# jianwang-mpi/GlobalEgoMocap

Hardware: AMD Instinct MI355X
Metric: optimised windows/sec (10-frame, 15-joint) (higher is better)
Workload: dtype f32

## Files before the change

### __graft_entry__.py

```python
import os
import subprocess
import sys

ROOT = os.path.dirname(os.path.abspath(__file__))
if ROOT not in sys.path:
    sys.path.insert(0, ROOT)

CSRC = os.path.join(ROOT, "globalegomocap_amd", "csrc")
LIB_DIR = os.path.join(ROOT, "globalegomocap_amd", "_lib")
LIB = os.path.join(LIB_DIR, "libgem_hip.so")
SOURCES = ["gem_api.hip", "weights.hip", "stage.hip", "gemm_f32.hip", "gemm_bf16.hip", "decoder_bf16.hip", "energy.hip", "lbfgs.hip", "tail.hip", "tail_bf16.hip", "train.hip", "errors.hip", "chunk_io.hip"]


def _stale():
    if not os.path.exists(LIB):
        return True
    t = os.path.getmtime(LIB)
    deps = [os.path.join(CSRC, f) for f in os.listdir(CSRC)] + [os.path.join(ROOT, "include", "gem_hip.h"),
                                                                os.path.abspath(__file__)]
    return any(os.path.getmtime(d) > t for d in deps)


NO_PACKED_FP32 = ["-Xclang", "-target-feature", "-Xclang", "-packed-fp32-ops", "-DGEM_NO_PACKED_FP32"]
FP_CONTRACT = ["-ffp-contract=on"]
EXTRA_FLAGS = {}
OBJ_DIR = os.path.join(ROOT, "build", "obj")
# ... 172 lines not shown
```

### globalegomocap_amd/csrc/energy.hip

```cpp
#include "energy_device.h"

namespace gem {

__global__ void pack_pose_kernel(const float* __restrict__ src, float* __restrict__ dst, int rows, int C) {
    const int i = blockIdx.x * blockDim.x + threadIdx.x;
    if (i >= rows * PAD) return;
    const int r = i / PAD, c = i % PAD;
    dst[i] = c < C ? src[(size_t)r * C + c] : 0.f;
}
__global__ void unpack_pose_kernel(const float* __restrict__ src, float* __restrict__ dst, int rows, int C) {
    const int i = blockIdx.x * blockDim.x + threadIdx.x;
    if (i >= rows * C) return;
    const int r = i / C, c = i % C;
    dst[i] = src[(size_t)r * PAD + c];
}
int launch_pack_pose(const float* src, float* dst, int rows, int C, hipStream_t s) {
    const int n = rows * PAD;
    hipLaunchKernelGGL(pack_pose_kernel, dim3((n + 255) / 256), dim3(256), 0, s, src, dst, rows, C);
    GEM_HIP(hipGetLastError());
    return 0;
}
int launch_unpack_pose(const float* src, float* dst, int rows, int C, hipStream_t s) {
    const int n = rows * C;
    hipLaunchKernelGGL(unpack_pose_kernel, dim3((n + 255) / 256), dim3(256), 0, s, src, dst, rows, C);
    GEM_HIP(hipGetLastError());
    return 0;
}

__global__ void reparam_kernel(const float* __restrict__ mulv, const float* __restrict__ eps, float* mu, float* logvar,
                               float* z, float* z2, int B, int D, int Dp) {
    const int i = blockIdx.x * blockDim.x + threadIdx.x;
    if (i >= B * Dp) return;
    const int b = i / Dp, k = i % Dp;
    float m = 0.f, lv = 0.f, zz = 0.f;
    if (k < D) {
        m = mulv[(size_t)b * 2 * Dp + k];
        lv = mulv[(size_t)b * 2 * Dp + Dp + k];
        zz = eps ? eps[(size_t)b * D + k] * expf(0.5f * lv) + m : m;
        if (mu) mu[(size_t)b * D + k] = m;
        if (logvar) logvar[(size_t)b * D + k] = lv;
        if (z) z[(size_t)b * D + k] = zz;
    }
    if (z2) z2[i] = zz;
}
int launch_reparam(const float* mulv, const float* eps, float* mu, float* logvar, float* z, float* z2, int B, int D, int Dp,
                   hipStream_t s) {
    const int n = B * Dp;
    hipLaunchKernelGGL(reparam_kernel, dim3((n + 255) / 256), dim3(256), 0, s, mulv, eps, mu, logvar, z, z2, B, D, Dp);
    GEM_HIP(hipGetLastError());
    return 0;
}
__global__ void pad_latent_kernel(const float* __restrict__ z, float* __restrict__ zp, int B, int D, int Dp) {
    const int i = blockIdx.x * blockDim.x + threadIdx.x;
// ... 81 lines not shown

__global__ void gather_windows_kernel(const float* __restrict__ frames, const int32_t* __restrict__ frame0,
                                      float* __restrict__ out, int B, int T, int JC) {
    const int i = blockIdx.x * blockDim.x + threadIdx.x;
    if (i >= B * T * JC) return;
    const int b = i / (T * JC), r = i - b * T * JC;
    out[i] = frames[(size_t)frame0[b] * JC + r];
}
int launch_gather_windows(const float* frames, const int32_t* frame0, float* out, int B, int T, int JC, hipStream_t s) {
    const int n = B * T * JC;
    hipLaunchKernelGGL(gather_windows_kernel, dim3((n + 255) / 256), dim3(256), 0, s, frames, frame0, out, B, T, JC);
    GEM_HIP(hipGetLastError());
    return 0;
}

__device__ void inv4_rigid_general(const double* m, double* o) {
    const double a = m[0], b = m[1], c = m[2], d = m[4], e = m[5], f = m[6], g = m[8], hh = m[9], i = m[10];
    const double A = e * i - f * hh, Bc = -(d * i - f * g), Cc = d * hh - e * g;
    const double det = a * A + b * Bc + c * Cc;
    const double id = 1.0 / det;
    double r[9] = {A * id, -(b * i - c * hh) * id, (b * f - c * e) * id,
                   Bc * id, (a * i - c * g) * id, -(a * f - c * d) * id,
                   Cc * id, -(a * hh - b * g) * id, (a * e - b * d) * id};
    const double tx = m[3], ty = m[7], tz = m[11];
    for (int q = 0; q < 3; ++q) {
        o[q * 4 + 0] = r[q * 3 + 0]; o[q * 4 + 1] = r[q * 3 + 1]; o[q * 4 + 2] = r[q * 3 + 2];
        o[q * 4 + 3] = -(r[q * 3 + 0] * tx + r[q * 3 + 1] * ty + r[q * 3 + 2] * tz);
    }
    o[12] = 0; o[13] = 0; o[14] = 0; o[15] = 1;
}

__global__ __launch_bounds__(64) void relative_global_kernel(const float* __restrict__ local, const double* __restrict__ cams,
                                                             const int32_t* __restrict__ frame0, float* __restrict__ rel,
                                                             int T, int J) {
    __shared__ double M[MAXT][12];
    const int b = blockIdx.x, lane = threadIdx.x;
    const double* c0 = cams + (size_t)frame0[b] * 16;
    if (lane < T) {
        double inv0[16];
        inv4_rigid_general(c0, inv0);
        const double* ct = c0 + (size_t)lane * 16;
        for (int r = 0; r < 3; ++r)
            for (int c = 0; c < 4; ++c) {
                double acc = 0;
                for (int k = 0; k < 4; ++k) acc += inv0[r * 4 + k] * ct[k * 4 + c];
                M[lane][r * 4 + c] = acc;
            }
    }
    __syncthreads();
    for (int p = lane; p < T * J; p += 64) {
        const int t = p / J;
        const float* x = local + ((size_t)b * T * J + p) * 3;
        const double X = x[0], Y = x[1], Z = x[2];
        float* o = rel + ((size_t)b * T * J + p) * 3;
        for (int r = 0; r < 3; ++r)
            o[r] = (float)(M[t][r * 4 + 0] * X + M[t][r * 4 + 1] * Y + M[t][r * 4 + 2] * Z + M[t][r * 4 + 3]);
    }
}
__global__ __launch_bounds__(64) void to_global_kernel(const float* __restrict__ rel, const double* __restrict__ cams,
                                                       const int32_t* __restrict__ frame0, double* __restrict__ out, int T, int J) {
    const int b = blockIdx.x, lane = threadIdx.x;
    const double* c0 = cams + (size_t)frame0[b] * 16;
    for (int p = lane; p < T * J; p += 64) {
        const float* x = rel + ((size_t)b * T * J + p) * 3;
        const double X = x[0], Y = x[1], Z = x[2];
        double* o = out + ((size_t)b * T * J + p) * 3;
        for (int r = 0; r < 3; ++r) o[r] = c0[r * 4 + 0] * X + c0[r * 4 + 1] * Y + c0[r * 4 + 2] * Z + c0[r * 4 + 3];
    }
}
int launch_relative_global(const float* local, const double* cams, const int32_t* frame0, float* rel, int B, int T, int J,
                           hipStream_t s) {
    hipLaunchKernelGGL(relative_global_kernel, dim3(B), dim3(64), 0, s, local, cams, frame0, rel, T, J);
    GEM_HIP(hipGetLastError());
    return 0;
}
int launch_to_global(const float* rel, const double* cams, const int32_t* frame0, double* out, int B, int T, int J,
                     hipStream_t s) {
    hipLaunchKernelGGL(to_global_kernel, dim3(B), dim3(64), 0, s, rel, cams, frame0, out, T, J);
    GEM_HIP(hipGetLastError());
    return 0;
}

}
// ... 1 lines not shown
```

### globalegomocap_amd/csrc/gem_internal.h

```cpp
#pragma once
#if defined(__HIP_DEVICE_COMPILE__) && !defined(GEM_NO_PACKED_FP32)
#error "compile with: -Xclang -target-feature -Xclang -packed-fp32-ops -DGEM_NO_PACKED_FP32 (__graft_entry__.NO_PACKED_FP32)"
#endif

#include <hip/hip_runtime.h>
#include <stdint.h>
#include <atomic>
#include <set>
#include <string>
#include <vector>

#include "../../include/gem_hip.h"

namespace gem {

constexpr int PAD = 64;
constexpr float LEAKY_SLOPE = 0.01f;
constexpr double BN_EPS = 1e-5;
constexpr int MAX_HIST = 128;
constexpr int MAXJ_ERR = GEM_MAX_JOINTS;
constexpr int N_LOG = 1 << 16;
constexpr int TRACE_ROUNDS = 64;

inline int pad64(int x) { return (x + PAD - 1) / PAD * PAD; }
// ... 77 lines not shown
    double* parts = nullptr;
    int* tex_key = nullptr;
    float* tex_val = nullptr;
    double* trace = nullptr;
    float* pose_a = nullptr;
    float* pose_b = nullptr;
    float* splitk = nullptr;
    size_t splitk_elems = 0;
    int* perm = nullptr;
    int* slot_of = nullptr;
    int* n_active = nullptr;
    int *perm2 = nullptr, *slot_of2 = nullptr;
    int* n_log = nullptr;
    long log_pos = 0;
    int done_phase = 3;
    int dbg_slots = -1, dbg_B = 0, dbg_round = 0;
    long dbg_log0 = 0;
    std::vector<void*> allocs;
};

enum Repack {
    REPACK_NONE = 0,
    REPACK_KERNEL = 1,
    REPACK_FUSED = 2,
    REPACK_ATOMIC = 3
};

struct RoundSet {
    int* n_active = nullptr;
    int* perm = nullptr;
// ... 70 lines not shown
}
__device__ __forceinline__ double wave_max_dpp(double v) {
    v = nan_max(v, dpp_move<0xB1>(v));
    v = nan_max(v, dpp_move<0x4E>(v));
    v = nan_max(v, dpp_move<0x141>(v));
    v = nan_max(v, dpp_move<0x140>(v));
    return nan_max(nan_max(nan_max(read_lane(v, 0), read_lane(v, 16)), read_lane(v, 32)), read_lane(v, 48));
}

}

namespace gem {
struct GraphKey {
    int kind = 0, stage = 0, B = 0, precision = 0;
    bool tex_cache = true;
    const void* ptr[12] = {};
    gem_energy_weights w[2] = {};
    gem_lbfgs_opts opt = {};
    void* stream = nullptr;
};
struct GraphEntry {
    GraphKey key;
    hipGraph_t graph = nullptr;
    hipGraphExec_t exec = nullptr;
    uint64_t last_use = 0;
};
}

struct gem_handle {
    gem_config cfg;
// ... 163 lines not shown
int launch_relative_global(const float* local, const double* cams, const int32_t* frame0, float* rel, int B, int T, int J,
                           hipStream_t s);
int launch_to_global(const float* rel, const double* cams, const int32_t* frame0, double* out, int B, int T, int J,
                     hipStream_t s);

int launch_errors(gem_handle* h, const double* est, const double* mid, const double* opt, const double* gt, int F,
                  const double* bone_mm, double* frame_out, double* out, hipStream_t s, int n_seq);
int launch_merge(const double* win, double* tmp, double* out, int n_chunks, int wpc, int T, int JC, int overlap, int smooth,
                 hipStream_t s);
size_t errors_frame_lds_bytes(int J);
void drop_graphs(gem_handle* h);
int post_scratch(gem_handle* h, size_t elems);
int launch_lift(gem_handle* h, const float* heat, const double* depth, int F, const double* poly, int n_poly, int up, int pad_x,
                int pad_y, double* out64, float* out32, hipStream_t s);

int launch_lbfgs_init(gem_handle* h, int B, hipStream_t s);
int launch_lbfgs_advance(gem_handle* h, int B, const gem_lbfgs_opts& o, const RoundSet& rs, const SlabSrc& grad, hipStream_t s);
int launch_lbfgs_stats(gem_handle* h, int B, gem_window_stats* out, hipStream_t s);
int launch_compact(gem_handle* h, const RoundSet& rs, int B, int force_all, hipStream_t s, int zero_after = 0);
int launch_lbfgs_debug_read(gem_handle* h, int B, gem_lbfgs_debug_state* out, float* x, float* d, float* trial, hipStream_t s);


}
```

### globalegomocap_amd/csrc/lbfgs.hip

```cpp
#include "gem_internal.h"

namespace gem {

typedef float f32x4 __attribute__((ext_vector_type(4)));

enum { PH_INIT = 0, PH_BRACKET = 1, PH_ZOOM = 2, PH_DONE = 3 };
static_assert(PH_DONE == 3, "Workspace::done_phase (gem_internal.h) names this value for the fused compaction of gemm_rows.h");

struct AdvArgs {
    LbfgsState* state;
    const double* f;
    double* trace;
    const float* gnew;
    float *x, *d, *g, *gp, *bg0, *bg1, *trial, *S, *Y;
    uint16_t* trial_b;
    int* phase_arr;
    const int* slot_of;
    int *next_perm, *next_slot_of, *next_count;
    SlabSrc gslab;
    unsigned long long* clk;
    int Dp, hist_cap;
    gem_lbfgs_opts o;
};

// ... 563 lines not shown
    }
#endif
    (void)full_path;
#undef LB_PROBE
}

template <int EPT, bool FULL, bool HB = false>
__global__ __launch_bounds__(256) void lbfgs_advance_kernel(AdvArgs a) { lbfgs_advance_body<EPT, 256, FULL, HB>(a); }

__global__ void lbfgs_init_kernel(LbfgsState* st, int* __restrict__ phase_arr, const float* __restrict__ trial, float* __restrict__ x, int B,
                                  int Dp) {
    const size_t i = (size_t)blockIdx.x * blockDim.x + threadIdx.x;
    if (i < (size_t)B * Dp) x[i] = trial[i];
    if (i < (size_t)B) {
        phase_arr[i] = PH_INIT;
        LbfgsState* s = st + i;
        s->phase = PH_INIT; s->n_iter = 0; s->evals = 0; s->ls_iter = 0; s->ls_evals = 0; s->max_ls = 0;
        s->first_bracket = 0; s->ls_done = 0; s->insuf = 0; s->low = 0; s->high = 1; s->hist_count = 0; s->hist_start = 0;
        s->nan_seen = 0;
        s->loss = 0; s->prev_loss = 0; s->t = 0; s->gtd = 0; s->d_norm = 0; s->H_diag = 1;
        s->t_prev = 0; s->f_prev = 0; s->gtd_prev = 0;
        s->br_t[0] = s->br_t[1] = 0; s->br_f[0] = s->br_f[1] = 0; s->br_gtd[0] = s->br_gtd[1] = 0;
    }
}

__global__ void lbfgs_stats_kernel(const LbfgsState* st, gem_window_stats* out, int B) {
    const int i = blockIdx.x * blockDim.x + threadIdx.x;
    if (i >= B) return;
    out[i].n_iter = st[i].n_iter;
    out[i].func_evals = st[i].evals;
    out[i].final_loss = (float)st[i].loss;
    out[i].status = (st[i].phase == PH_DONE ? 1 : 0) | (st[i].nan_seen ? 2 : 0);
}

__global__ __launch_bounds__(256) void lbfgs_debug_read_kernel(const LbfgsState* __restrict__ st, gem_lbfgs_debug_state* __restrict__ out,
                                                               const float* __restrict__ x, const float* __restrict__ d,
                                                               const float* __restrict__ trial, const uint16_t* __restrict__ trial_b,
                                                               float* __restrict__ ox, float* __restrict__ od, float* __restrict__ otrial,
                                                               int D, int Dp) {
    __shared__ int bad;
    const int b = blockIdx.x;
    if (threadIdx.x == 0) bad = 0;
    __syncthreads();
    int mine = 0;
    for (int k = threadIdx.x; k < Dp; k += blockDim.x) {
        const size_t i = (size_t)b * Dp + k;
        const float xv = x[i], dv = d[i];
// ... 137 lines not shown
```

### globalegomocap_amd/csrc/stage.hip

```cpp
#include <cstring>

#include "gem_internal.h"

namespace gem {

__global__ void fill_u32_kernel(uint32_t* __restrict__ p, uint32_t v, size_t n) {
    const size_t i = (size_t)blockIdx.x * blockDim.x + threadIdx.x;
    if (i < n) p[i] = v;
}
static int launch_fill_u32(uint32_t* p, uint32_t v, size_t n, hipStream_t s) {
    if (!n) return 0;
    hipLaunchKernelGGL(fill_u32_kernel, dim3((unsigned)((n + 255) / 256)), dim3(256), 0, s, p, v, n);
    GEM_HIP(hipGetLastError());
    return 0;
}


Route plan_route(const gem_handle* h, int stage, int B, Call call) {
    const StageNet& net = h->net[stage];
    Route rt;
    rt.precision = h->precision;
    const bool bf16 = h->precision == GEM_PRECISION_BF16, have_tail = net.tail_start >= 1;
    const int tail_g = h->T <= 16 ? 16 / h->T : 1;
    rt.tail_wgs = (B + tail_g - 1) / tail_g;
// ... 29 lines not shown
    const bool odd = mode == REPACK_ATOMIC && (k & 1);
    r.perm = odd ? w.perm2 : w.perm;
    r.slot_of = mode == REPACK_NONE ? nullptr : odd ? w.slot_of2 : w.slot_of;
    r.n_active = w.n_active;
    r.log_idx = log0 + k;
    if (mode == REPACK_ATOMIC) {
        r.n_active = w.n_log + (log0 + k) % N_LOG;
        r.next_count = r.n_active + 1;
        r.next_perm = odd ? w.perm : w.perm2;
        r.next_slot_of = odd ? w.slot_of : w.slot_of2;
    }
    r.trace = k < TRACE_ROUNDS ? w.trace + (size_t)k * w.Bmax : nullptr;
    return r;
}

static int begin_rounds(gem_handle* h, int B, int counters, hipStream_t s, long* log0) {
    Workspace& w = h->ws;
    if (counters && (w.log_pos % N_LOG) + counters + 1 > N_LOG) w.log_pos += N_LOG - (w.log_pos % N_LOG);
    *log0 = w.log_pos;
    if (launch_compact(h, round_set(w, *log0, 0, REPACK_KERNEL), B, 1, s, counters)) return 1;
    w.log_pos = *log0 + 1 + counters;
    return 0;
}

static int check_lbfgs_opts(const Workspace& w, const gem_lbfgs_opts& o, const char* who) {
    if (o.max_iter < 1 || o.max_eval < 1 || o.max_iter - 1 > w.hist_cap || o.max_iter > MAX_HIST) {
        set_error(std::string(who) + ": max_iter must be 1.." + std::to_string(w.hist_cap + 1)); return 1;
    }
    if (o.max_eval > 1021) { set_error(std::string(who) + ": max_eval must be at most 1021 (torch's default for max_iter = 25 is 31)"); return 1; }
    return 0;
}

static int check_call(gem_handle* h, int stage, int B, const char* who) {
    if (!h) { set_error(std::string(who) + ": null handle"); return 1; }
    if (stage < 0 || stage > 1 || !h->net[stage].loaded) { set_error(std::string(who) + ": VAE weights of this stage are not loaded"); return 1; }
    if (B < 0 || B > h->ws.Bmax) { set_error(std::string(who) + ": B exceeds max_windows"); return 1; }
    GEM_HIP(hipSetDevice(h->cfg.device));
    return 0;
}

static int encoder_forward(gem_handle* h, int stage, int B, const float* d_pose, hipStream_t s) {
    StageNet& net = h->net[stage];
    Workspace& w = h->ws;
    const int rows = B * h->T;
    if (launch_pack_pose(d_pose, w.pose_p, rows, h->C, s)) return 1;
    const float* in = w.pose_p;
    int lda = PAD;
    for (size_t i = 0; i < net.enc.size(); ++i) {
        if (launch_gemm(h, net.enc[i], EPI_BIAS_LRELU, in, lda, nullptr, w.enc_act[i], net.enc[i].N, rows, h->T, s, -1)) return 1;
        in = w.enc_act[i];
        lda = net.enc[i].N;
    }
    return launch_gemm(h, net.fc, EPI_BIAS, in, net.fc.K, nullptr, w.mulv, net.fc.N, B, h->T, s, -1);
}


static int decoder_forward(gem_handle* h, const Route& rt, int stage, int B, const float* zp, hipStream_t s, const RoundSet* rs = nullptr,
                           int* repack_log = nullptr) {
    StageNet& net = h->net[stage];
    Workspace& w = h->ws;
// ... 98 lines not shown
    fill_tail_args(h, net, rt, B, forward_only, in_slab, ea, rs, &ta);
    ta.g_out = w.dec_grad[st]; ta.g_out_b = nullptr;
    if (launch_tail(h, ta, tail_lds, s, rs)) return 1;
    if (forward_only) return 0;
    return decoder_backward(h, rt, stage, B, s, st - 1, w.dec_grad[st], rs, grad);
}

struct StageRun {
    gem_handle* h = nullptr;
    int stage = 0, B = 0;
    const float* pose_in = nullptr; const float* heat = nullptr; const int32_t* frame0 = nullptr; const float* mean_bone = nullptr;
    const float* eps = nullptr;
    gem_energy_weights wt{}; gem_lbfgs_opts opt{};
    float* pose_out = nullptr; gem_window_stats* stats = nullptr;
    hipStream_t s = nullptr;
    EnergyArgs ea{};
    Route route;
    long log0 = 0;
    int rounds = 0;
};

static int stage_begin(StageRun& r) {
    gem_handle* h = r.h;
    Workspace& w = h->ws;
    const int B = r.B, stage = r.stage;
    hipStream_t s = r.s;
    if (r.wt.reproj != 0.0 && (!r.heat || !r.frame0)) { set_error("optimize: reproj weight != 0 needs heat-maps and frame indices"); return 1; }
    if (check_lbfgs_opts(w, r.opt, "optimize")) return 1;
    r.rounds = r.opt.max_eval + 1;
    w.dbg_slots = -1;
    if (encoder_forward(h, stage, B, r.pose_in, s)) return 1;
    if (launch_reparam(w.mulv, r.eps, nullptr, nullptr, nullptr, w.trial, B, h->D, h->Dp, s)) return 1;
    if (h->precision == GEM_PRECISION_BF16 && launch_f32_to_bf16(w.trial, w.trial_b, (size_t)B * h->Dp, s)) return 1;
    if (launch_lbfgs_init(h, B, s)) return 1;
    r.route = plan_route(h, stage, B, CALL_ROUNDS);
    if (begin_rounds(h, B, r.route.repack == REPACK_ATOMIC ? r.rounds + 1 : 0, s, &r.log0)) return 1;
    const bool tex = h->tex_cache && w.tex_key && r.wt.reproj != 0.0;
    if (tex && launch_fill_u32(reinterpret_cast<uint32_t*>(w.tex_key), 0xFFFFFFFFu, (size_t)B * h->T * h->J, s)) return 1;
    r.ea = energy_args(h, r.pose_in, r.heat, r.frame0, r.mean_bone, r.wt, tex);
    return launch_fill_u32(reinterpret_cast<uint32_t*>(w.trace), 0xFFFFFFFFu, (size_t)TRACE_ROUNDS * w.Bmax * 2, s);
}

static int stage_round(StageRun& r, int k) {
    gem_handle* h = r.h;
    Workspace& w = h->ws;
    const Repack mode = r.route.repack;
    const RoundSet rs = round_set(w, r.log0, k, mode);
    int* repack_log = nullptr;
    if (k > 0 && mode != REPACK_ATOMIC) {
        if (mode == REPACK_FUSED) repack_log = w.n_log + rs.log_idx % N_LOG;
        else if (launch_compact(h, rs, r.B, 0, r.s)) return 1;
        w.log_pos = rs.log_idx + 1;
    }
    r.ea.n_dev = rs.n_active; r.ea.perm = rs.perm;
    SlabSrc grad;
    if (evaluate(h, r.route, r.stage, r.B, w.trial, r.ea, r.s, false, &rs, &grad, repack_log)) return 1;
    return launch_lbfgs_advance(h, r.B, r.opt, rs, grad, r.s);
}

static int stage_finish(StageRun& r) {
    gem_handle* h = r.h;
    Workspace& w = h->ws;
    SlabSrc none;
    if (evaluate(h, r.route, r.stage, r.B, w.trial, energy_args(h, r.pose_in, r.heat, r.frame0, r.mean_bone, r.wt, false), r.s, true, nullptr, &none))
        return 1;
    if (launch_unpack_pose(w.dec_act.back(), r.pose_out, r.B * h->T, h->C, r.s)) return 1;
    if (r.stats && launch_lbfgs_stats(h, r.B, r.stats, r.s)) return 1;
    return 0;
}

static int optimize_stage_impl(gem_handle* h, int stage, int B, const float* d_pose_in, const float* d_heat,
                               const int32_t* d_frame0, const float* d_mean_bone, const float* d_eps,
                               const gem_energy_weights& wt, const gem_lbfgs_opts& opt, float* d_pose_out,
                               gem_window_stats* d_stats, hipStream_t s) {
    StageRun r;
    r.h = h; r.stage = stage; r.B = B; r.pose_in = d_pose_in; r.heat = d_heat; r.frame0 = d_frame0; r.mean_bone = d_mean_bone; r.eps = d_eps;
    r.wt = wt; r.opt = opt; r.pose_out = d_pose_out; r.stats = d_stats; r.s = s;
    int rc = stage_begin(r);
    for (int k = 0; k < r.rounds && !rc; ++k) rc = stage_round(r, k);
    return rc || stage_finish(r);
}

struct WindowsRun {
    gem_handle* h = nullptr;
    int B = 0;
    const float* local_pose = nullptr; const double* cams = nullptr; const float* heat = nullptr; const int32_t* frame0 = nullptr;
    const float* mean_bone = nullptr; const float* eps_local = nullptr; const float* eps_global = nullptr;
    gem_energy_weights w_local{}, w_global{}; gem_lbfgs_opts opt{};
    float* mid_local = nullptr; double* global = nullptr; gem_window_stats* stats_local = nullptr; gem_window_stats* stats_global = nullptr;
    hipStream_t s = nullptr;
    StageRun st;
    float* mid = nullptr;
};

static int windows_begin_local(WindowsRun& r) {
    gem_handle* h = r.h;
    Workspace& w = h->ws;
    if (launch_gather_windows(r.local_pose, r.frame0, w.pose_a, r.B, h->T, h->C, r.s)) return 1;
    r.mid = r.mid_local ? r.mid_local : w.pose_b;
    StageRun& s = r.st;
    s = StageRun{};
    s.h = h; s.stage = GEM_STAGE_LOCAL; s.B = r.B; s.pose_in = w.pose_a; s.heat = r.heat; s.frame0 = r.frame0; s.mean_bone = r.mean_bone;
    s.eps = r.eps_local; s.wt = r.w_local; s.opt = r.opt; s.pose_out = r.mid; s.stats = r.stats_local; s.s = r.s;
    return stage_begin(s);
}
static int windows_begin_global(WindowsRun& r) {
    gem_handle* h = r.h;
    Workspace& w = h->ws;
    if (stage_finish(r.st)) return 1;
    if (launch_relative_global(r.mid, r.cams, r.frame0, w.pose_a, r.B, h->T, h->J, r.s)) return 1;
    StageRun& s = r.st;
    s = StageRun{};
    s.h = h; s.stage = GEM_STAGE_GLOBAL; s.B = r.B; s.pose_in = w.pose_a; s.heat = r.heat; s.frame0 = r.frame0; s.mean_bone = r.mean_bone;
    s.eps = r.eps_global; s.wt = r.w_global; s.opt = r.opt; s.pose_out = w.pose_b;
    s.stats = r.stats_global; s.s = r.s;
    return stage_begin(s);
}
static int windows_end(WindowsRun& r) {
    gem_handle* h = r.h;
    if (stage_finish(r.st)) return 1;
    return launch_to_global(h->ws.pose_b, r.cams, r.frame0, r.global, r.B, h->T, h->J, r.s);
}

static int windows_single(WindowsRun& r) {
    int rc = windows_begin_local(r);
    for (int k = 0; k < r.st.rounds && !rc; ++k) rc = stage_round(r.st, k);
    rc = rc || windows_begin_global(r);
    for (int k = 0; k < r.st.rounds && !rc; ++k) rc = stage_round(r.st, k);
    return rc || windows_end(r);
}

static bool same_key(const GraphKey& a, const GraphKey& b) {
    if (a.kind != b.kind || a.stage != b.stage || a.B != b.B || a.precision != b.precision || a.stream != b.stream || a.tex_cache != b.tex_cache)
        return false;
    for (int i = 0; i < 12; ++i)
        if (a.ptr[i] != b.ptr[i]) return false;
    return std::memcmp(a.w, b.w, sizeof(a.w)) == 0 && std::memcmp(&a.opt, &b.opt, sizeof(a.opt)) == 0;
}

template <typename Body>
static int run_graphed(gem_handle* h, const GraphKey& key, hipStream_t s, Body body) {
    if (!h->graphs_on || s == nullptr || h->prof.on) return body();
    GraphEntry* e = nullptr;
    for (auto& g : h->graphs)
        if (same_key(g.key, key)) { e = &g; break; }
    ++h->graph_tick;
    if (!e) {
        if (h->graphs.size() >= 16) {
// ... 26 lines not shown
    ++h->graph_replays;
    return 0;
}

}

using namespace gem;

extern "C" {

int gem_encode(gem_handle* h, int stage, int B, const float* d_pose, const float* d_eps, float* d_mu, float* d_logvar,
               float* d_z, void* stream) {
    if (check_call(h, stage, B, "gem_encode")) return 1;
    hipStream_t s = (hipStream_t)stream;
    if (B == 0) return 0;
    if (encoder_forward(h, stage, B, d_pose, s)) return 1;
    return launch_reparam(h->ws.mulv, d_eps, d_mu, d_logvar, d_z, nullptr, B, h->D, h->Dp, s);
}

int gem_decode(gem_handle* h, int stage, int B, const float* d_z, float* d_pose, void* stream) {
    if (check_call(h, stage, B, "gem_decode")) return 1;
    hipStream_t s = (hipStream_t)stream;
    if (B == 0) return 0;
    if (launch_pad_latent(d_z, h->ws.trial, B, h->D, h->Dp, s)) return 1;
    if (decoder_forward(h, plan_route(h, stage, B, CALL_DECODE), stage, B, h->ws.trial, s)) return 1;
    return launch_unpack_pose(h->ws.dec_act.back(), d_pose, B * h->T, h->C, s);
}

int gem_energy_grad(gem_handle* h, int stage, int B, const float* d_z, const float* d_pose_init, const float* d_heat,
                    const int32_t* d_frame0, const float* d_mean_bone, const gem_energy_weights* wt, double* d_energy,
                    double* d_parts, float* d_dz, float* d_pose, void* stream) {
// ... 32 lines not shown
    });
}

int gem_optimize_windows(gem_handle* h, int B, const float* d_local_pose, const double* d_cams, const float* d_heat,
                         const int32_t* d_frame0, const float* d_mean_bone, const float* d_eps_local, const float* d_eps_global,
                         const gem_energy_weights* w_local, const gem_energy_weights* w_global, const gem_lbfgs_opts* opt,
                         float* d_mid_local, double* d_global, gem_window_stats* d_stats, void* stream) {
    if (check_call(h, 0, B, "gem_optimize_windows") || check_call(h, 1, B, "gem_optimize_windows")) return 1;
    if (B == 0) return 0;
    if (!d_local_pose || !d_cams || !d_frame0 || !d_mean_bone || !w_local || !w_global || !opt || !d_global) {
        set_error("gem_optimize_windows: null argument"); return 1;
    }
    hipStream_t s = (hipStream_t)stream;
    GraphKey key;
    key.kind = 2; key.B = B; key.precision = h->precision; key.stream = stream; key.tex_cache = h->tex_cache;
    const void* ptrs[] = {d_local_pose, d_cams, d_heat, d_frame0, d_mean_bone, d_eps_local, d_eps_global, d_mid_local, d_global, d_stats};
    for (int i = 0; i < 10; ++i) key.ptr[i] = ptrs[i];
    key.w[0] = *w_local; key.w[1] = *w_global; key.opt = *opt;
    return run_graphed(h, key, s, [&]() -> int {
        WindowsRun a;
        a.h = h; a.B = B; a.local_pose = d_local_pose; a.cams = d_cams; a.heat = d_heat; a.frame0 = d_frame0; a.mean_bone = d_mean_bone;
        a.eps_local = d_eps_local; a.eps_global = d_eps_global; a.w_local = *w_local; a.w_global = *w_global; a.opt = *opt;
        a.mid_local = d_mid_local; a.global = d_global; a.stats_local = d_stats; a.stats_global = d_stats ? d_stats + B : nullptr; a.s = s;
        return windows_single(a);
    });
}

int gem_read_trace(gem_handle* h, int B, int n_rounds, double* d_out, void* stream) {
    if (!h || !d_out || B < 0 || B > h->ws.Bmax || n_rounds < 0 || n_rounds > TRACE_ROUNDS) {
        set_error("gem_read_trace: need 0 <= B <= max_windows and 0 <= n_rounds <= 64"); return 1;
    }
    GEM_HIP(hipSetDevice(h->cfg.device));
    if (B == 0 || n_rounds == 0) return 0;
    GEM_HIP(hipMemcpy2DAsync(d_out, (size_t)B * sizeof(double), h->ws.trace, (size_t)h->ws.Bmax * sizeof(double),
                             (size_t)B * sizeof(double), (size_t)n_rounds, hipMemcpyDeviceToDevice, (hipStream_t)stream));
    return 0;
}

// ... 72 lines not shown
```

Baseline: 32060.

## Fuse stage-boundary kernels: gather+pack, begin init, finish+frame transforms

Adds fused kernels at the boundaries between the local and global optimisation stages. A single gather_pack kernel replaces the separate gather and pack launches. One stage_begin kernel folds together reparameterisation, L-BFGS state reset, compaction init, counter zeroing, tex-key fill and trace fill. A stage_finish kernel merges unpack, stats, and the relative/global camera transforms, including repacking the next stage's padded input. The aim is fewer small kernel launches and graph nodes plus fewer global round-trips. In exchange there is more code complexity and a larger one-dimensional grid in stage_begin that is sized by the biggest fill.

```diff
diff --git a/__graft_entry__.py b/__graft_entry__.py
--- a/__graft_entry__.py
+++ b/__graft_entry__.py
@@ -9,7 +9,7 @@
 CSRC = os.path.join(ROOT, "globalegomocap_amd", "csrc")
 LIB_DIR = os.path.join(ROOT, "globalegomocap_amd", "_lib")
 LIB = os.path.join(LIB_DIR, "libgem_hip.so")
-SOURCES = ["gem_api.hip", "weights.hip", "stage.hip", "gemm_f32.hip", "gemm_bf16.hip", "decoder_bf16.hip", "energy.hip", "lbfgs.hip", "tail.hip", "tail_bf16.hip", "train.hip", "errors.hip", "chunk_io.hip"]
+SOURCES = ["gem_api.hip", "weights.hip", "stage.hip", "gemm_f32.hip", "gemm_bf16.hip", "decoder_bf16.hip", "energy.hip", "stage_boundary.hip", "lbfgs.hip", "tail.hip", "tail_bf16.hip", "train.hip", "errors.hip", "chunk_io.hip"]
 
 
 def _stale():
diff --git a/globalegomocap_amd/csrc/energy.hip b/globalegomocap_amd/csrc/energy.hip
--- a/globalegomocap_amd/csrc/energy.hip
+++ b/globalegomocap_amd/csrc/energy.hip
@@ -1,4 +1,5 @@
 #include "energy_device.h"
+#include "stage_boundary.h"
 
 namespace gem {
 
@@ -36,7 +37,7 @@
     if (k < D) {
         m = mulv[(size_t)b * 2 * Dp + k];
         lv = mulv[(size_t)b * 2 * Dp + Dp + k];
-        zz = eps ? eps[(size_t)b * D + k] * expf(0.5f * lv) + m : m;
+        zz = eps ? reparam_z(m, lv, eps[(size_t)b * D + k]) : m;
         if (mu) mu[(size_t)b * D + k] = m;
         if (logvar) logvar[(size_t)b * D + k] = lv;
         if (z) z[(size_t)b * D + k] = zz;
@@ -148,59 +149,18 @@
     return 0;
 }
 
-__device__ void inv4_rigid_general(const double* m, double* o) {
-    const double a = m[0], b = m[1], c = m[2], d = m[4], e = m[5], f = m[6], g = m[8], hh = m[9], i = m[10];
-    const double A = e * i - f * hh, Bc = -(d * i - f * g), Cc = d * hh - e * g;
-    const double det = a * A + b * Bc + c * Cc;
-    const double id = 1.0 / det;
-    double r[9] = {A * id, -(b * i - c * hh) * id, (b * f - c * e) * id,
-                   Bc * id, (a * i - c * g) * id, -(a * f - c * d) * id,
-                   Cc * id, -(a * hh - b * g) * id, (a * e - b * d) * id};
-    const double tx = m[3], ty = m[7], tz = m[11];
-    for (int q = 0; q < 3; ++q) {
-        o[q * 4 + 0] = r[q * 3 + 0]; o[q * 4 + 1] = r[q * 3 + 1]; o[q * 4 + 2] = r[q * 3 + 2];
-        o[q * 4 + 3] = -(r[q * 3 + 0] * tx + r[q * 3 + 1] * ty + r[q * 3 + 2] * tz);
-    }
-    o[12] = 0; o[13] = 0; o[14] = 0; o[15] = 1;
-}
-
 __global__ __launch_bounds__(64) void relative_global_kernel(const float* __restrict__ local, const double* __restrict__ cams,
                                                              const int32_t* __restrict__ frame0, float* __restrict__ rel,
                                                              int T, int J) {
     __shared__ double M[MAXT][12];
-    const int b = blockIdx.x, lane = threadIdx.x;
-    const double* c0 = cams + (size_t)frame0[b] * 16;
-    if (lane < T) {
-        double inv0[16];
-        inv4_rigid_general(c0, inv0);
-        const double* ct = c0 + (size_t)lane * 16;
-        for (int r = 0; r < 3; ++r)
-            for (int c = 0; c < 4; ++c) {
-                double acc = 0;
-                for (int k = 0; k < 4; ++k) acc += inv0[r * 4 + k] * ct[k * 4 + c];
-                M[lane][r * 4 + c] = acc;
-            }
-    }
-    __syncthreads();
-    for (int p = lane; p < T * J; p += 64) {
-        const int t = p / J;
-        const float* x = local + ((size_t)b * T * J + p) * 3;
-        const double X = x[0], Y = x[1], Z = x[2];
-        float* o = rel + ((size_t)b * T * J + p) * 3;
-        for (int r = 0; r < 3; ++r)
-            o[r] = (float)(M[t][r * 4 + 0] * X + M[t][r * 4 + 1] * Y + M[t][r * 4 + 2] * Z + M[t][r * 4 + 3]);
-    }
+    const int b = blockIdx.x;
+    relative_global_window(local + (size_t)b * T * J * 3, J * 3, cams + (size_t)frame0[b] * 16, rel + (size_t)b * T * J * 3, T, J,
+                           threadIdx.x, M);
 }
 __global__ __launch_bounds__(64) void to_global_kernel(const float* __restrict__ rel, const double* __restrict__ cams,
                                                        const int32_t* __restrict__ frame0, double* __restrict__ out, int T, int J) {
-    const int b = blockIdx.x, lane = threadIdx.x;
-    const double* c0 = cams + (size_t)frame0[b] * 16;
-    for (int p = lane; p < T * J; p += 64) {
-        const float* x = rel + ((size_t)b * T * J + p) * 3;
-        const double X = x[0], Y = x[1], Z = x[2];
-        double* o = out + ((size_t)b * T * J + p) * 3;
-        for (int r = 0; r < 3; ++r) o[r] = c0[r * 4 + 0] * X + c0[r * 4 + 1] * Y + c0[r * 4 + 2] * Z + c0[r * 4 + 3];
-    }
+    const int b = blockIdx.x;
+    to_global_window(rel + (size_t)b * T * J * 3, J * 3, cams + (size_t)frame0[b] * 16, out + (size_t)b * T * J * 3, T, J, threadIdx.x);
 }
 int launch_relative_global(const float* local, const double* cams, const int32_t* frame0, float* rel, int B, int T, int J,
                            hipStream_t s) {
diff --git a/globalegomocap_amd/csrc/gem_internal.h b/globalegomocap_amd/csrc/gem_internal.h
--- a/globalegomocap_amd/csrc/gem_internal.h
+++ b/globalegomocap_amd/csrc/gem_internal.h
@@ -115,6 +115,7 @@
     int* n_log = nullptr;
     long log_pos = 0;
     int done_phase = 3;
+    int init_phase = 0;
     int dbg_slots = -1, dbg_B = 0, dbg_round = 0;
     long dbg_log0 = 0;
     std::vector<void*> allocs;
@@ -215,6 +216,7 @@
 struct GraphKey {
     int kind = 0, stage = 0, B = 0, precision = 0;
     bool tex_cache = true;
+    bool fused_boundary = false;
     const void* ptr[12] = {};
     gem_energy_weights w[2] = {};
     gem_lbfgs_opts opt = {};
@@ -408,6 +410,30 @@
 int launch_lift(gem_handle* h, const float* heat, const double* depth, int F, const double* poly, int n_poly, int up, int pad_x,
                 int pad_y, double* out64, float* out32, hipStream_t s);
 
+struct StageBeginArgs {
+    const float* mulv; const float* eps;
+    float* trial; float* x;
+    LbfgsState* state; int* phase;
+    int *perm, *slot_of, *n_active, *log_slot;
+    uint32_t* tex_key; size_t tex_n;
+    uint32_t* trace; size_t trace_n;
+    int B, D, Dp, T, init_phase, zero_after;
+};
+enum BoundaryTransform { BOUNDARY_NONE = 0, BOUNDARY_RELATIVE = 1, BOUNDARY_TO_GLOBAL = 2 };
+struct StageFinishArgs {
+    const float* Xp;
+    float* pose_out;
+    const LbfgsState* state; gem_window_stats* stats;
+    const double* cams; const int32_t* frame0;
+    float* rel;
+    float* next_padded;
+    double* glob;
+    int T, J, done_phase, transform;
+};
+int launch_gather_pack(const float* frames, const int32_t* frame0, float* dense, float* padded, int B, int T, int C, hipStream_t s);
+int launch_stage_begin(const StageBeginArgs& a, hipStream_t s);
+int launch_stage_finish(const StageFinishArgs& a, int B, hipStream_t s);
+
 int launch_lbfgs_init(gem_handle* h, int B, hipStream_t s);
 int launch_lbfgs_advance(gem_handle* h, int B, const gem_lbfgs_opts& o, const RoundSet& rs, const SlabSrc& grad, hipStream_t s);
 int launch_lbfgs_stats(gem_handle* h, int B, gem_window_stats* out, hipStream_t s);
diff --git a/globalegomocap_amd/csrc/lbfgs.hip b/globalegomocap_amd/csrc/lbfgs.hip
--- a/globalegomocap_amd/csrc/lbfgs.hip
+++ b/globalegomocap_amd/csrc/lbfgs.hip
@@ -1,4 +1,5 @@
 #include "gem_internal.h"
+#include "stage_boundary.h"
 
 namespace gem {
 
@@ -6,6 +7,7 @@
 
 enum { PH_INIT = 0, PH_BRACKET = 1, PH_ZOOM = 2, PH_DONE = 3 };
 static_assert(PH_DONE == 3, "Workspace::done_phase (gem_internal.h) names this value for the fused compaction of gemm_rows.h");
+static_assert(PH_INIT == 0, "Workspace::init_phase (gem_internal.h) names this value for stage_begin_kernel (stage_boundary.hip)");
 
 struct AdvArgs {
     LbfgsState* state;
@@ -601,23 +603,14 @@
     if (i < (size_t)B * Dp) x[i] = trial[i];
     if (i < (size_t)B) {
         phase_arr[i] = PH_INIT;
-        LbfgsState* s = st + i;
-        s->phase = PH_INIT; s->n_iter = 0; s->evals = 0; s->ls_iter = 0; s->ls_evals = 0; s->max_ls = 0;
-        s->first_bracket = 0; s->ls_done = 0; s->insuf = 0; s->low = 0; s->high = 1; s->hist_count = 0; s->hist_start = 0;
-        s->nan_seen = 0;
-        s->loss = 0; s->prev_loss = 0; s->t = 0; s->gtd = 0; s->d_norm = 0; s->H_diag = 1;
-        s->t_prev = 0; s->f_prev = 0; s->gtd_prev = 0;
-        s->br_t[0] = s->br_t[1] = 0; s->br_f[0] = s->br_f[1] = 0; s->br_gtd[0] = s->br_gtd[1] = 0;
+        lbfgs_reset_window(st + i, PH_INIT);
     }
 }
 
 __global__ void lbfgs_stats_kernel(const LbfgsState* st, gem_window_stats* out, int B) {
     const int i = blockIdx.x * blockDim.x + threadIdx.x;
     if (i >= B) return;
-    out[i].n_iter = st[i].n_iter;
-    out[i].func_evals = st[i].evals;
-    out[i].final_loss = (float)st[i].loss;
-    out[i].status = (st[i].phase == PH_DONE ? 1 : 0) | (st[i].nan_seen ? 2 : 0);
+    window_stats(st[i], out + i, PH_DONE);
 }
 
 __global__ __launch_bounds__(256) void lbfgs_debug_read_kernel(const LbfgsState* __restrict__ st, gem_lbfgs_debug_state* __restrict__ out,
diff --git a/globalegomocap_amd/csrc/stage.hip b/globalegomocap_amd/csrc/stage.hip
--- a/globalegomocap_amd/csrc/stage.hip
+++ b/globalegomocap_amd/csrc/stage.hip
@@ -67,13 +67,26 @@
     return r;
 }
 
-static int begin_rounds(gem_handle* h, int B, int counters, hipStream_t s, long* log0) {
+static int begin_rounds(gem_handle* h, int B, int counters, hipStream_t s, long* log0, StageBeginArgs* fused = nullptr) {
     Workspace& w = h->ws;
     if (counters && (w.log_pos % N_LOG) + counters + 1 > N_LOG) w.log_pos += N_LOG - (w.log_pos % N_LOG);
     *log0 = w.log_pos;
-    if (launch_compact(h, round_set(w, *log0, 0, REPACK_KERNEL), B, 1, s, counters)) return 1;
+    const RoundSet r0 = round_set(w, *log0, 0, REPACK_KERNEL);
+    if (fused) {
+        const long slot = r0.log_idx % N_LOG;
+        if (counters < 0 || counters > 1024 || slot + counters >= N_LOG) { set_error("stage_begin: bad counter range"); return 1; }
+        fused->perm = r0.perm; fused->slot_of = r0.slot_of; fused->n_active = r0.n_active; fused->log_slot = w.n_log + slot;
+        fused->zero_after = counters;
+    } else if (launch_compact(h, r0, B, 1, s, counters)) {
+        return 1;
+    }
     w.log_pos = *log0 + 1 + counters;
     return 0;
+}
+
+static bool fused_boundary_on() {
+    const char* e = dev_env("GEM_FUSED_BOUNDARY");
+    return !(e && e[0] == '0');
 }
 
 static int check_lbfgs_opts(const Workspace& w, const gem_lbfgs_opts& o, const char* who) {
@@ -92,11 +105,16 @@
     return 0;
 }
 
-static int encoder_forward(gem_handle* h, int stage, int B, const float* d_pose, hipStream_t s) {
+static int encoder_forward(gem_handle* h, int stage, int B, float* d_pose_gathered, const float* d_pose, hipStream_t s,
+                           const float* gather_frames = nullptr, const int32_t* gather_frame0 = nullptr, bool packed = false) {
     StageNet& net = h->net[stage];
     Workspace& w = h->ws;
     const int rows = B * h->T;
-    if (launch_pack_pose(d_pose, w.pose_p, rows, h->C, s)) return 1;
+    if (gather_frames) {
+        if (launch_gather_pack(gather_frames, gather_frame0, d_pose_gathered, w.pose_p, B, h->T, h->C, s)) return 1;
+    } else if (!packed && launch_pack_pose(d_pose, w.pose_p, rows, h->C, s)) {
+        return 1;
+    }
     const float* in = w.pose_p;
     int lda = PAD;
     for (size_t i = 0; i < net.enc.size(); ++i) {
@@ -225,6 +243,10 @@
     gem_energy_weights wt{}; gem_lbfgs_opts opt{};
     float* pose_out = nullptr; gem_window_stats* stats = nullptr;
     hipStream_t s = nullptr;
+    bool fused = false;
+    const float* gather_frames = nullptr; float* pose_in_w = nullptr;
+    bool pose_in_packed = false;
+    int transform = BOUNDARY_NONE; const double* cams = nullptr; float* rel_out = nullptr; double* glob_out = nullptr;
     EnergyArgs ea{};
     Route route;
     long log0 = 0;
@@ -240,13 +262,26 @@
     if (check_lbfgs_opts(w, r.opt, "optimize")) return 1;
     r.rounds = r.opt.max_eval + 1;
     w.dbg_slots = -1;
-    if (encoder_forward(h, stage, B, r.pose_in, s)) return 1;
+    r.route = plan_route(h, stage, B, CALL_ROUNDS);
+    const bool tex = h->tex_cache && w.tex_key && r.wt.reproj != 0.0;
+    if (r.fused) {
+        if (encoder_forward(h, stage, B, r.pose_in_w, r.pose_in, s, r.gather_frames, r.frame0, r.pose_in_packed)) return 1;
+        StageBeginArgs b{};
+        b.mulv = w.mulv; b.eps = r.eps; b.trial = w.trial; b.x = w.x; b.state = w.state; b.phase = w.phase;
+        b.B = B; b.D = h->D; b.Dp = h->Dp; b.T = h->T; b.init_phase = w.init_phase;
+        if (begin_rounds(h, B, r.route.repack == REPACK_ATOMIC ? r.rounds + 1 : 0, s, &r.log0, &b)) return 1;
+        b.tex_key = reinterpret_cast<uint32_t*>(w.tex_key); b.tex_n = tex ? (size_t)B * h->T * h->J : 0;
+        b.trace = reinterpret_cast<uint32_t*>(w.trace); b.trace_n = (size_t)TRACE_ROUNDS * w.Bmax * 2;
+        if (launch_stage_begin(b, s)) return 1;
+        if (h->precision == GEM_PRECISION_BF16 && launch_f32_to_bf16(w.trial, w.trial_b, (size_t)B * h->Dp, s)) return 1;
+        r.ea = energy_args(h, r.pose_in, r.heat, r.frame0, r.mean_bone, r.wt, tex);
+        return 0;
+    }
+    if (encoder_forward(h, stage, B, nullptr, r.pose_in, s)) return 1;
     if (launch_reparam(w.mulv, r.eps, nullptr, nullptr, nullptr, w.trial, B, h->D, h->Dp, s)) return 1;
     if (h->precision == GEM_PRECISION_BF16 && launch_f32_to_bf16(w.trial, w.trial_b, (size_t)B * h->Dp, s)) return 1;
     if (launch_lbfgs_init(h, B, s)) return 1;
-    r.route = plan_route(h, stage, B, CALL_ROUNDS);
     if (begin_rounds(h, B, r.route.repack == REPACK_ATOMIC ? r.rounds + 1 : 0, s, &r.log0)) return 1;
-    const bool tex = h->tex_cache && w.tex_key && r.wt.reproj != 0.0;
     if (tex && launch_fill_u32(reinterpret_cast<uint32_t*>(w.tex_key), 0xFFFFFFFFu, (size_t)B * h->T * h->J, s)) return 1;
     r.ea = energy_args(h, r.pose_in, r.heat, r.frame0, r.mean_bone, r.wt, tex);
     return launch_fill_u32(reinterpret_cast<uint32_t*>(w.trace), 0xFFFFFFFFu, (size_t)TRACE_ROUNDS * w.Bmax * 2, s);
@@ -275,6 +310,13 @@
     SlabSrc none;
     if (evaluate(h, r.route, r.stage, r.B, w.trial, energy_args(h, r.pose_in, r.heat, r.frame0, r.mean_bone, r.wt, false), r.s, true, nullptr, &none))
         return 1;
+    if (r.fused) {
+        StageFinishArgs f{};
+        f.Xp = w.dec_act.back(); f.pose_out = r.pose_out; f.state = w.state; f.stats = r.stats;
+        f.cams = r.cams; f.frame0 = r.frame0; f.rel = r.rel_out; f.next_padded = w.pose_p; f.glob = r.glob_out;
+        f.T = h->T; f.J = h->J; f.done_phase = w.done_phase; f.transform = r.transform;
+        return launch_stage_finish(f, r.B, r.s);
+    }
     if (launch_unpack_pose(w.dec_act.back(), r.pose_out, r.B * h->T, h->C, r.s)) return 1;
     if (r.stats && launch_lbfgs_stats(h, r.B, r.stats, r.s)) return 1;
     return 0;
@@ -302,15 +344,20 @@
     hipStream_t s = nullptr;
     StageRun st;
     float* mid = nullptr;
+    bool fused = false;
 };
 
 static int windows_begin_local(WindowsRun& r) {
     gem_handle* h = r.h;
     Workspace& w = h->ws;
-    if (launch_gather_windows(r.local_pose, r.frame0, w.pose_a, r.B, h->T, h->C, r.s)) return 1;
+    if (!r.fused && launch_gather_windows(r.local_pose, r.frame0, w.pose_a, r.B, h->T, h->C, r.s)) return 1;
     r.mid = r.mid_local ? r.mid_local : w.pose_b;
     StageRun& s = r.st;
     s = StageRun{};
+    if (r.fused) {
+        s.fused = true; s.gather_frames = r.local_pose; s.pose_in_w = w.pose_a;
+        s.transform = BOUNDARY_RELATIVE; s.cams = r.cams; s.rel_out = w.pose_a;
+    }
     s.h = h; s.stage = GEM_STAGE_LOCAL; s.B = r.B; s.pose_in = w.pose_a; s.heat = r.heat; s.frame0 = r.frame0; s.mean_bone = r.mean_bone;
     s.eps = r.eps_local; s.wt = r.w_local; s.opt = r.opt; s.pose_out = r.mid; s.stats = r.stats_local; s.s = r.s;
     return stage_begin(s);
@@ -319,9 +366,10 @@
     gem_handle* h = r.h;
     Workspace& w = h->ws;
     if (stage_finish(r.st)) return 1;
-    if (launch_relative_global(r.mid, r.cams, r.frame0, w.pose_a, r.B, h->T, h->J, r.s)) return 1;
+    if (!r.fused && launch_relative_global(r.mid, r.cams, r.frame0, w.pose_a, r.B, h->T, h->J, r.s)) return 1;
     StageRun& s = r.st;
     s = StageRun{};
+    if (r.fused) { s.fused = true; s.pose_in_packed = true; s.transform = BOUNDARY_TO_GLOBAL; s.cams = r.cams; s.glob_out = r.global; }
     s.h = h; s.stage = GEM_STAGE_GLOBAL; s.B = r.B; s.pose_in = w.pose_a; s.heat = r.heat; s.frame0 = r.frame0; s.mean_bone = r.mean_bone;
     s.eps = r.eps_global; s.wt = r.w_global; s.opt = r.opt; s.pose_out = w.pose_b;
     s.stats = r.stats_global; s.s = r.s;
@@ -330,7 +378,7 @@
 static int windows_end(WindowsRun& r) {
     gem_handle* h = r.h;
     if (stage_finish(r.st)) return 1;
-    return launch_to_global(h->ws.pose_b, r.cams, r.frame0, r.global, r.B, h->T, h->J, r.s);
+    return r.fused ? 0 : launch_to_global(h->ws.pose_b, r.cams, r.frame0, r.global, r.B, h->T, h->J, r.s);
 }
 
 static int windows_single(WindowsRun& r) {
@@ -342,7 +390,8 @@
 }
 
 static bool same_key(const GraphKey& a, const GraphKey& b) {
-    if (a.kind != b.kind || a.stage != b.stage || a.B != b.B || a.precision != b.precision || a.stream != b.stream || a.tex_cache != b.tex_cache)
+    if (a.kind != b.kind || a.stage != b.stage || a.B != b.B || a.precision != b.precision || a.stream != b.stream || a.tex_cache != b.tex_cache ||
+        a.fused_boundary != b.fused_boundary)
         return false;
     for (int i = 0; i < 12; ++i)
         if (a.ptr[i] != b.ptr[i]) return false;
@@ -399,7 +448,7 @@
     if (check_call(h, stage, B, "gem_encode")) return 1;
     hipStream_t s = (hipStream_t)stream;
     if (B == 0) return 0;
-    if (encoder_forward(h, stage, B, d_pose, s)) return 1;
+    if (encoder_forward(h, stage, B, nullptr, d_pose, s)) return 1;
     return launch_reparam(h->ws.mulv, d_eps, d_mu, d_logvar, d_z, nullptr, B, h->D, h->Dp, s);
 }
 
@@ -462,6 +511,7 @@
     hipStream_t s = (hipStream_t)stream;
     GraphKey key;
     key.kind = 2; key.B = B; key.precision = h->precision; key.stream = stream; key.tex_cache = h->tex_cache;
+    key.fused_boundary = fused_boundary_on() && h->C == h->J * 3;
     const void* ptrs[] = {d_local_pose, d_cams, d_heat, d_frame0, d_mean_bone, d_eps_local, d_eps_global, d_mid_local, d_global, d_stats};
     for (int i = 0; i < 10; ++i) key.ptr[i] = ptrs[i];
     key.w[0] = *w_local; key.w[1] = *w_global; key.opt = *opt;
@@ -470,6 +520,7 @@
         a.h = h; a.B = B; a.local_pose = d_local_pose; a.cams = d_cams; a.heat = d_heat; a.frame0 = d_frame0; a.mean_bone = d_mean_bone;
         a.eps_local = d_eps_local; a.eps_global = d_eps_global; a.w_local = *w_local; a.w_global = *w_global; a.opt = *opt;
         a.mid_local = d_mid_local; a.global = d_global; a.stats_local = d_stats; a.stats_global = d_stats ? d_stats + B : nullptr; a.s = s;
+        a.fused = key.fused_boundary;
         return windows_single(a);
     });
 }
diff --git a/globalegomocap_amd/csrc/stage_boundary.h b/globalegomocap_amd/csrc/stage_boundary.h
--- /dev/null
+++ b/globalegomocap_amd/csrc/stage_boundary.h
@@ -0,0 +1,74 @@
+#pragma once
+#include "gem_internal.h"
+
+namespace gem {
+
+__device__ __forceinline__ float reparam_z(float m, float lv, float e) { return e * expf(0.5f * lv) + m; }
+
+__device__ __forceinline__ void lbfgs_reset_window(LbfgsState* s, int init_phase) {
+    s->phase = init_phase; s->n_iter = 0; s->evals = 0; s->ls_iter = 0; s->ls_evals = 0; s->max_ls = 0;
+    s->first_bracket = 0; s->ls_done = 0; s->insuf = 0; s->low = 0; s->high = 1; s->hist_count = 0; s->hist_start = 0;
+    s->nan_seen = 0;
+    s->loss = 0; s->prev_loss = 0; s->t = 0; s->gtd = 0; s->d_norm = 0; s->H_diag = 1;
+    s->t_prev = 0; s->f_prev = 0; s->gtd_prev = 0;
+    s->br_t[0] = s->br_t[1] = 0; s->br_f[0] = s->br_f[1] = 0; s->br_gtd[0] = s->br_gtd[1] = 0;
+}
+
+__device__ __forceinline__ void window_stats(const LbfgsState& s, gem_window_stats* out, int done_phase) {
+    out->n_iter = s.n_iter;
+    out->func_evals = s.evals;
+    out->final_loss = (float)s.loss;
+    out->status = (s.phase == done_phase ? 1 : 0) | (s.nan_seen ? 2 : 0);
+}
+
+__device__ inline void inv4_rigid_general(const double* m, double* o) {
+    const double a = m[0], b = m[1], c = m[2], d = m[4], e = m[5], f = m[6], g = m[8], hh = m[9], i = m[10];
+    const double A = e * i - f * hh, Bc = -(d * i - f * g), Cc = d * hh - e * g;
+    const double det = a * A + b * Bc + c * Cc;
+    const double id = 1.0 / det;
+    double r[9] = {A * id, -(b * i - c * hh) * id, (b * f - c * e) * id,
+                   Bc * id, (a * i - c * g) * id, -(a * f - c * d) * id,
+                   Cc * id, -(a * hh - b * g) * id, (a * e - b * d) * id};
+    const double tx = m[3], ty = m[7], tz = m[11];
+    for (int q = 0; q < 3; ++q) {
+        o[q * 4 + 0] = r[q * 3 + 0]; o[q * 4 + 1] = r[q * 3 + 1]; o[q * 4 + 2] = r[q * 3 + 2];
+        o[q * 4 + 3] = -(r[q * 3 + 0] * tx + r[q * 3 + 1] * ty + r[q * 3 + 2] * tz);
+    }
+    o[12] = 0; o[13] = 0; o[14] = 0; o[15] = 1;
+}
+
+__device__ __forceinline__ void relative_global_window(const float* __restrict__ src, int ld, const double* __restrict__ c0,
+                                                       float* __restrict__ rel, int T, int J, int lane, double (*M)[12]) {
+    if (lane < T) {
+        double inv0[16];
+        inv4_rigid_general(c0, inv0);
+        const double* ct = c0 + (size_t)lane * 16;
+        for (int r = 0; r < 3; ++r)
+            for (int c = 0; c < 4; ++c) {
+                double acc = 0;
+                for (int k = 0; k < 4; ++k) acc += inv0[r * 4 + k] * ct[k * 4 + c];
+                M[lane][r * 4 + c] = acc;
+            }
+    }
+    __syncthreads();
+    for (int p = lane; p < T * J; p += 64) {
+        const int t = p / J;
+        const float* x = src + (size_t)t * ld + (p - t * J) * 3;
+        const double X = x[0], Y = x[1], Z = x[2];
+        float* o = rel + (size_t)p * 3;
+        for (int r = 0; r < 3; ++r)
+            o[r] = (float)(M[t][r * 4 + 0] * X + M[t][r * 4 + 1] * Y + M[t][r * 4 + 2] * Z + M[t][r * 4 + 3]);
+    }
+}
+__device__ __forceinline__ void to_global_window(const float* __restrict__ src, int ld, const double* __restrict__ c0,
+                                                 double* __restrict__ out, int T, int J, int lane) {
+    for (int p = lane; p < T * J; p += 64) {
+        const int t = p / J;
+        const float* x = src + (size_t)t * ld + (p - t * J) * 3;
+        const double X = x[0], Y = x[1], Z = x[2];
+        double* o = out + (size_t)p * 3;
+        for (int r = 0; r < 3; ++r) o[r] = c0[r * 4 + 0] * X + c0[r * 4 + 1] * Y + c0[r * 4 + 2] * Z + c0[r * 4 + 3];
+    }
+}
+
+}
diff --git a/globalegomocap_amd/csrc/stage_boundary.hip b/globalegomocap_amd/csrc/stage_boundary.hip
--- /dev/null
+++ b/globalegomocap_amd/csrc/stage_boundary.hip
@@ -0,0 +1,93 @@
+#include "energy_device.h"
+#include "stage_boundary.h"
+
+namespace gem {
+
+__global__ void gather_pack_kernel(const float* __restrict__ frames, const int32_t* __restrict__ frame0, float* __restrict__ dense,
+                                   float* __restrict__ padded, int B, int T, int C) {
+    const int i = blockIdx.x * blockDim.x + threadIdx.x;
+    if (i >= B * T * PAD) return;
+    const int row = i / PAD, c = i % PAD;
+    const int b = row / T, t = row - b * T;
+    float v = 0.f;
+    if (c < C) {
+        v = frames[((size_t)frame0[b] + t) * C + c];
+        dense[(size_t)row * C + c] = v;
+    }
+    padded[i] = v;
+}
+
+int launch_gather_pack(const float* frames, const int32_t* frame0, float* dense, float* padded, int B, int T, int C, hipStream_t s) {
+    const int n = B * T * PAD;
+    hipLaunchKernelGGL(gather_pack_kernel, dim3((n + 255) / 256), dim3(256), 0, s, frames, frame0, dense, padded, B, T, C);
+    GEM_HIP(hipGetLastError());
+    return 0;
+}
+
+__global__ __launch_bounds__(256) void stage_begin_kernel(const StageBeginArgs a) {
+    const size_t i = (size_t)blockIdx.x * blockDim.x + threadIdx.x;
+    if (i < (size_t)a.B * a.Dp) {
+        const int b = (int)(i / a.Dp), k = (int)(i % a.Dp);
+        float zz = 0.f;
+        if (k < a.D) {
+            const float m = a.mulv[(size_t)b * 2 * a.Dp + k];
+            const float lv = a.mulv[(size_t)b * 2 * a.Dp + a.Dp + k];
+            zz = a.eps ? reparam_z(m, lv, a.eps[(size_t)b * a.D + k]) : m;
+        }
+        a.trial[i] = zz;
+        a.x[i] = zz;
+    }
+    if (i < (size_t)a.B) {
+        a.phase[i] = a.init_phase;
+        lbfgs_reset_window(a.state + i, a.init_phase);
+        a.perm[i] = (int)i;
+        a.slot_of[i] = (int)i;
+    }
+    if (i == 0) { a.n_active[0] = a.B; a.n_active[1] = a.B * a.T; *a.log_slot = a.B; }
+    if (i < (size_t)a.zero_after) a.log_slot[1 + i] = 0;
+    if (i < a.tex_n) a.tex_key[i] = 0xFFFFFFFFu;
+    if (i < a.trace_n) a.trace[i] = 0xFFFFFFFFu;
+}
+
+int launch_stage_begin(const StageBeginArgs& a, hipStream_t s) {
+    if (a.zero_after < 0 || a.zero_after > 1024) { set_error("stage_begin: bad counter range"); return 1; }
+    size_t n = (size_t)a.B * a.Dp;
+    if (a.tex_n > n) n = a.tex_n;
+    if (a.trace_n > n) n = a.trace_n;
+    if ((size_t)a.zero_after > n) n = (size_t)a.zero_after;
+    hipLaunchKernelGGL(stage_begin_kernel, dim3((unsigned)((n + 255) / 256)), dim3(256), 0, s, a);
+    GEM_HIP(hipGetLastError());
+    return 0;
+}
+
+__global__ __launch_bounds__(64) void stage_finish_kernel(const StageFinishArgs a) {
+    __shared__ double M[MAXT][12];
+    const int b = blockIdx.x, lane = threadIdx.x;
+    const int T = a.T, J = a.J, C = J * 3;
+    const float* Xp = a.Xp + (size_t)b * T * PAD;
+    for (int p = lane; p < T * C; p += 64) {
+        const int t = p / C;
+        a.pose_out[(size_t)b * T * C + p] = Xp[(size_t)t * PAD + (p - t * C)];
+    }
+    if (lane == 0 && a.stats) window_stats(a.state[b], a.stats + b, a.done_phase);
+    if (a.transform == BOUNDARY_RELATIVE) {
+        float* rel = a.rel + (size_t)b * T * C;
+        relative_global_window(Xp, PAD, a.cams + (size_t)a.frame0[b] * 16, rel, T, J, lane, M);
+        __syncthreads();
+        float* padded = a.next_padded + (size_t)b * T * PAD;
+        for (int i = lane; i < T * PAD; i += 64) {
+            const int t = i / PAD, c = i % PAD;
+            padded[i] = c < C ? rel[(size_t)t * C + c] : 0.f;
+        }
+    } else if (a.transform == BOUNDARY_TO_GLOBAL)
+        to_global_window(Xp, PAD, a.cams + (size_t)a.frame0[b] * 16, a.glob + (size_t)b * T * C, T, J, lane);
+}
+
+int launch_stage_finish(const StageFinishArgs& a, int B, hipStream_t s) {
+    if (a.T > MAXT || a.J * 3 > PAD) { set_error("stage_finish: T <= 16 and J*3 <= 64 supported"); return 1; }
+    hipLaunchKernelGGL(stage_finish_kernel, dim3(B), dim3(64), 0, s, a);
+    GEM_HIP(hipGetLastError());
+    return 0;
+}
+
+}
```

Measured after the change: 32180 (median of 6 runs). No clear change (+0.4%).
